# OpenResearchInstitute/ka9q-sdr

Measured on AMD Instinct MI355X. Metric: input Msamples/s + channels @ real-time, 16384-pt overlap-save, higher is better.
Workload: dtype f32

## Files before the change

### ka9q_sdr_amd/csrc/kq_demod64.hip

```cpp
#include "kq_device.hpp"
#include <cstdlib>
#include "kq_ldsfft.hpp"

namespace kq {

namespace {

__device__ __forceinline__ float2 shfl2(float2 v, int src) {
  return make_float2(__shfl(v.x, src, 64), __shfl(v.y, src, 64));
}
__device__ __forceinline__ float rdlane(float v, int src) {
  return __int_as_float(__builtin_amdgcn_readlane(__float_as_int(v), src));
}
__device__ __forceinline__ int bitrev6(int i) { return (int)(__brev((unsigned)i) >> 26); }

__device__ __forceinline__ void put_status(kq_chan_status &st, const Geom &g, const ChanDev &ch, const Planes &pl, int c, int b,
                                           int compute_n0, double n0_rate, float &n0) {
  st.if_power = pl.if_power[b];
  st.noise_gain = ch.noise_gain[c];
  st.plfreq = NAN;
  st.cphase = 0;
  st.pll_lock = 0;
  st.lock_count = 0;
  if (compute_n0) {
    float const fresh = pl.n0raw[(size_t)c * g.max_blocks + b];
    if (isnan(n0))
      n0 = fresh;
    else
      n0 = (float)((double)n0 + n0_rate * (double)(fresh - n0));
    st.n0 = n0;
  } else {
    st.n0 = NAN;
  }
}

template <class Op>
__device__ __forceinline__ float hreduce(float v, Op op) {
  int const lane = threadIdx.x & 63;
  v = op(v, lane_xor<16>(v, lane));
  v = op(v, lane_xor<8>(v, lane));
  v = op(v, lane_xor<4>(v, lane));
  v = op(v, lane_xor<2>(v, lane));
  v = op(v, lane_xor<1>(v, lane));
  return v;
}
__device__ __forceinline__ float hsum(float v) {
  return hreduce(v, [](float a, float b) { return a + b; });
}

template <bool FLAT>
__device__ void fm_channel_pair(const Geom &g, const ChanDev &ch, const Planes &pl, int c, int nblocks, int compute_n0) {
  int const lane = threadIdx.x & 63;
  int const h = lane >> 5, n = lane & 31;
  float const gain = ch.fm_gain[c];
  float const noise_gain = ch.noise_gain[c];
  int const kbin = bitrev6(lane);
  int const herm_src = bitrev6((64 - kbin) & 63);
  float2 HAf = make_float2(0.f, 0.f);
  if (!FLAT) {
    float2 const t = ch.aresp[(size_t)c * 33 + (kbin <= 32 ? kbin : 64 - kbin)];
    HAf = kbin <= 32 ? t : cconj(t);
  }
  bool const real_bin = kbin == 0 || kbin == 32;

  float2 wf[6], wi[6];
#pragma unroll
  for (int s = 0; s < 6; s++) {
    int const half = 1 << s;
    float sn, cs;
    sincospif((float)(lane & (half - 1)) / (float)half, &sn, &cs);
    wf[s] = make_float2(cs, -sn);
    wi[s] = make_float2(cs, sn);
  }

  float2 state = ch.fm_state[c];
  float lastaudio = ch.lastaudio[c];
  int sq = ch.sq_count[c];
  float foffset = ch.foffset[c], pdev = ch.pdev[c];
  float n0 = ch.n0[c];
  float hist = h ? 0.f : ch.ahist[(size_t)c * 32 + lane];
  float ifp_v = 0.f, n0raw_v = 0.f;
  const float2 *in = pl.filt + (size_t)c * g.max_blocks * 32;

  float2 s_next = (h < nblocks) ? in[lane] : make_float2(0.f, 0.f);
  for (int b = 0; b < nblocks; b += 2) {
    bool const have1 = b + 1 < nblocks;
    float2 const S = s_next;
    if (b + 2 < nblocks) s_next = (b + 2 + h < nblocks) ? in[(size_t)(b + 2) * 32 + lane] : make_float2(0.f, 0.f);
    if ((b & 63) == 0) {
      int const bb = b + lane;
      ifp_v = bb < nblocks ? pl.if_power[bb] : 0.f;
      n0raw_v = (compute_n0 && bb < nblocks) ? pl.n0raw[(size_t)c * g.max_blocks + bb] : 0.f;
    }

    float const t = cnrm(S);
    float const sum_t = hsum(t), sum_a = hsum(sqrtf(t));
    float const bbp = sum_t / 64.f;
    float const amp = (float)((double)sum_a / (M_SQRT2 * 32));
    float const variance = bbp - amp * amp;
    float snr = amp * amp / (2 * variance) - 1;
    snr = (0.0f > snr) ? 0.0f : snr;
    float const snr0 = rdlane(snr, 0), snr1 = rdlane(snr, 32);
    int nsq = sq + 1;
    nsq = nsq > 1000 ? 1000 : nsq;
    int const sq0 = (snr0 > 2) ? 0 : nsq;
    nsq = sq0 + 1;
    nsq = nsq > 1000 ? 1000 : nsq;
    int const sq1 = have1 ? ((snr1 > 2) ? 0 : nsq) : sq0;
    bool const open0 = sq0 < 2, open1 = have1 && sq1 < 2;
    bool const my_open = h ? open1 : open0;

    float const thr = (float)(0.55 * 0.55 * amp * amp);
    unsigned long long const raw = __ballot(t > thr);
    unsigned long long const m_lo = open0 ? (raw & 0xffffffffull) : 0ull;
    unsigned long long const m_hi = open1 ? (raw >> 32) : 0ull;
    unsigned long long const mask = m_lo | (m_hi << 32);
    bool const valid = (mask >> lane) & 1ull;
    unsigned long long const below = mask & ((1ull << lane) - 1ull);
    unsigned long long const upto = mask & ((2ull << lane) - 1ull);
    int const pv = below ? 63 - __clzll((long long)below) : -1;
    int const lv = upto ? 63 - __clzll((long long)upto) : -1;
    float2 const state_fb = (h && !open0) ? make_float2(0.f, 0.f) : state;
    float const la_fb = (h && !open0) ? 0.f : lastaudio;
    float2 const sp = shfl2(S, pv >= 0 ? pv : 0);
    float2 const stc = pv >= 0 ? cconj(sp) : state_fb;
    float2 const pr = cmul(S, stc);
    float const y = valid ? atan2f(pr.y, pr.x) : 0.f;
    float const yl = __shfl(y, lv >= 0 ? lv : 0, 64);
    float const out = my_open ? (lv >= 0 ? yl : la_fb) : 0.f;

    float const sum_y = hsum(out);
    float const vmax = hreduce((valid && n > 0) ? y : -INFINITY, [](float a, float b2) { return fmaxf(a, b2); });
    float const vmin = hreduce((valid && n > 0) ? y : INFINITY, [](float a, float b2) { return fminf(a, b2); });
    float const y_first = h ? rdlane(y, 32) : rdlane(y, 0);
    float const seed = ((mask >> (32 * h)) & 1ull) ? y_first : 0.f;
    float pdev_pos = fmaxf(seed, vmax), pdev_neg = fminf(seed, vmin);
    float const avg_f = sum_y / 32.f;
    pdev_pos -= avg_f;
    pdev_neg -= avg_f;
    float const mx = (pdev_pos > -pdev_neg) ? pdev_pos : -pdev_neg;
    float const fo_new = (float)(g.dsamprate * avg_f * (0.5 * M_1_PI));
    float const pd_new = (float)(g.dsamprate * mx * (0.5 * M_1_PI));
    float const fo0 = (sq0 < 1) ? rdlane(fo_new, 0) : foffset, pd0 = (sq0 < 1) ? rdlane(pd_new, 0) : pdev;
    float const fo1 = (have1 && sq1 < 1) ? rdlane(fo_new, 32) : fo0, pd1 = (have1 && sq1 < 1) ? rdlane(pd_new, 32) : pd0;

    {
      int const last0 = m_lo ? 63 - __clzll((long long)m_lo) : 0;
      int const last1 = m_hi ? 95 - __clzll((long long)m_hi) : 0;
      float2 const sl0 = cconj(make_float2(rdlane(S.x, last0), rdlane(S.y, last0)));
      float2 const sl1 = cconj(make_float2(rdlane(S.x, last1), rdlane(S.y, last1)));
      float const yl0 = rdlane(y, last0), yl1 = rdlane(y, last1);
      float2 st0 = open0 ? (m_lo ? sl0 : state) : make_float2(0.f, 0.f);
      float la0 = open0 ? (m_lo ? yl0 : lastaudio) : 0.f;
      if (have1) {
        st0 = open1 ? (m_hi ? sl1 : st0) : make_float2(0.f, 0.f);
        la0 = open1 ? (m_hi ? yl1 : la0) : 0.f;
      }
      state = st0;
      lastaudio = la0;
    }
    sq = sq1;
    foffset = fo1;
    pdev = pd1;

    float const xo = lane_xor<32>(out, lane);
    float a0 = out, a1 = xo;
    if (!FLAT) {
      float2 z = make_float2(h ? xo : hist, out);
#pragma unroll
      for (int s = 5; s >= 0; s--) {
        float2 const r = lane_xor_pow2(z, s, lane);
        z = ((lane >> s) & 1) ? cmul(csub(r, z), wf[s]) : cadd(z, r);
      }
      float2 const zm = cconj(shfl2(z, herm_src));
      float2 const z1 = make_float2(0.5f * (z.x + zm.x), 0.5f * (z.y + zm.y));
      float2 const z2 = make_float2(0.5f * (z.y - zm.y), -0.5f * (z.x - zm.x));
      float2 g1 = cmul(HAf, z1), g2 = cmul(HAf, z2);
      if (real_bin) g1.y = g2.y = 0.f;
      z = make_float2(g1.x - g2.y, g1.y + g2.x);
#pragma unroll
      for (int s = 0; s < 6; s++) {
        int const bit = (lane >> s) & 1;
        float2 const v = bit ? cmul(z, wi[s]) : z;
        float2 const r = lane_xor_pow2(v, s, lane);
        z = bit ? csub(r, v) : cadd(v, r);
      }
      a0 = z.x * gain;
      a1 = z.y * gain;
      if (h) {
        pl.audio[((size_t)c * g.max_blocks + b) * 64 + n] = a0;
        if (have1) pl.audio[((size_t)c * g.max_blocks + b + 1) * 64 + n] = a1;
      }
    } else {
      if (!h) {
        pl.audio[((size_t)c * g.max_blocks + b) * 64 + n] = a0;
        if (have1) pl.audio[((size_t)c * g.max_blocks + b + 1) * 64 + n] = a1;
      }
    }
    hist = have1 ? xo : out;

    float const ifp = h ? rdlane(ifp_v, (b + 1) & 63) : rdlane(ifp_v, b & 63);
    float const fresh0 = rdlane(n0raw_v, b & 63), fresh1 = rdlane(n0raw_v, (b + 1) & 63);
    float n0a = n0, n0b = n0;
    if (compute_n0) {
      n0a = isnan(n0) ? fresh0 : (float)((double)n0 + .01 * (double)(fresh0 - n0));
      n0b = have1 ? (isnan(n0a) ? fresh1 : (float)((double)n0a + .01 * (double)(fresh1 - n0a))) : n0a;
      n0 = n0b;
    }
    if (n == 0 && (h == 0 || have1)) {
      kq_chan_status rec;
      rec.if_power = ifp;
      rec.noise_gain = noise_gain;
      rec.plfreq = NAN;
      rec.cphase = 0;
      rec.pll_lock = 0;
      rec.lock_count = 0;
      rec.n0 = compute_n0 ? (h ? n0b : n0a) : NAN;
      rec.bb_power = bbp;
      rec.snr = snr;
      rec.foffset = h ? fo1 : fo0;
      rec.pdeviation = h ? pd1 : pd0;
      rec.agc_gain = 0;
      rec.squelch_count = h ? sq1 : sq0;
      rec.hangcount = 0;
      rec.blanked = my_open ? 32 - __popcll((mask >> (32 * h)) & 0xffffffffull) : 0;
      rec.nout = 32;
      pl.status[(size_t)c * g.max_blocks + b + h] = rec;
    }
  }
  if (!h) ch.ahist[(size_t)c * 32 + lane] = hist;
  if (lane == 0) {
    ch.fm_state[c] = state;
    ch.lastaudio[c] = lastaudio;
    ch.sq_count[c] = sq;
    ch.foffset[c] = foffset;
    ch.pdev[c] = pdev;
    ch.n0[c] = n0;
  }
}

__device__ void fm_channel_four_waves(const Geom &g, const ChanDev &ch, const Planes &pl, int c, int nblocks, int compute_n0) {
  __shared__ float2 s_S[2][64];
  __shared__ float s_a[2][2][4];
  __shared__ float s_out[2][64], s_y[2][64];
  __shared__ float s_b[2][2][5];
  __shared__ float2 s_z[2][64];
  __shared__ float s_c[2][2][6];
  int const lane = threadIdx.x & 63, role = threadIdx.x >> 6;
  int const h = lane >> 5, n = lane & 31;
  int const npairs = (nblocks + 1) / 2, niter = npairs + 3;

  if (role == 0) {
    int sq = ch.sq_count[c];
    const float2 *in = pl.filt + (size_t)c * g.max_blocks * 32;
    float2 s_next = (h < nblocks) ? in[lane] : make_float2(0.f, 0.f);
    for (int it = 0; it < niter; it++) {
      if (it < npairs) {
        int const b = 2 * it, par = it & 1;
        bool const have1 = b + 1 < nblocks;
        float2 const S = s_next;
        if (b + 2 < nblocks) s_next = (b + 2 + h < nblocks) ? in[(size_t)(b + 2) * 32 + lane] : make_float2(0.f, 0.f);
        float const t = cnrm(S);
        float const sum_t = hsum(t), sum_a = hsum(sqrtf(t));
        float const bbp = sum_t / 64.f;
        float const amp = (float)((double)sum_a / (M_SQRT2 * 32));
        float const variance = bbp - amp * amp;
        float snr = amp * amp / (2 * variance) - 1;
        snr = (0.0f > snr) ? 0.0f : snr;
        float const snr0 = rdlane(snr, 0), snr1 = rdlane(snr, 32);
        int nsq = sq + 1;
        nsq = nsq > 1000 ? 1000 : nsq;
        int const sq0 = (snr0 > 2) ? 0 : nsq;
        nsq = sq0 + 1;
        nsq = nsq > 1000 ? 1000 : nsq;
        int const sq1 = have1 ? ((snr1 > 2) ? 0 : nsq) : sq0;
        sq = sq1;
        s_S[par][lane] = S;
        if (n == 0) {
          float *st = s_a[par][h];
          st[0] = amp;
          st[1] = bbp;
          st[2] = snr;
          st[3] = __int_as_float(h ? sq1 : sq0);
        }
      }
      __syncthreads();
    }
    if (lane == 0) ch.sq_count[c] = sq;
    return;
  }

  if (role == 1) {
    float2 state = ch.fm_state[c];
    float lastaudio = ch.lastaudio[c];
    for (int it = 0; it < niter; it++) {
      if (it >= 1 && it - 1 < npairs) {
        int const b = 2 * (it - 1), par = (it - 1) & 1;
        bool const have1 = b + 1 < nblocks;
        float2 const S = s_S[par][lane];
        float const amp = s_a[par][h][0];
        int const sq0 = __float_as_int(s_a[par][0][3]), sq1 = __float_as_int(s_a[par][1][3]);
        bool const open0 = sq0 < 2, open1 = have1 && sq1 < 2;
        bool const my_open = h ? open1 : open0;
        float const t = cnrm(S);
        float const thr = (float)(0.55 * 0.55 * amp * amp);
        unsigned long long const raw = __ballot(t > thr);
        unsigned long long const m_lo = open0 ? (raw & 0xffffffffull) : 0ull;
        unsigned long long const m_hi = open1 ? (raw >> 32) : 0ull;
        unsigned long long const mask = m_lo | (m_hi << 32);
        bool const valid = (mask >> lane) & 1ull;
        unsigned long long const below = mask & ((1ull << lane) - 1ull);
        unsigned long long const upto = mask & ((2ull << lane) - 1ull);
        int const pv = below ? 63 - __clzll((long long)below) : -1;
        int const lv = upto ? 63 - __clzll((long long)upto) : -1;
        float2 const state_fb = (h && !open0) ? make_float2(0.f, 0.f) : state;
        float const la_fb = (h && !open0) ? 0.f : lastaudio;
        float2 const sp = shfl2(S, pv >= 0 ? pv : 0);
        float2 const stc = pv >= 0 ? cconj(sp) : state_fb;
        float2 const pr = cmul(S, stc);
        float const y = valid ? atan2f(pr.y, pr.x) : 0.f;
        float const yl = __shfl(y, lv >= 0 ? lv : 0, 64);
        float const out = my_open ? (lv >= 0 ? yl : la_fb) : 0.f;
        {
          int const last0 = m_lo ? 63 - __clzll((long long)m_lo) : 0;
          int const last1 = m_hi ? 95 - __clzll((long long)m_hi) : 0;
          float2 const sl0 = cconj(make_float2(rdlane(S.x, last0), rdlane(S.y, last0)));
          float2 const sl1 = cconj(make_float2(rdlane(S.x, last1), rdlane(S.y, last1)));
          float const yl0 = rdlane(y, last0), yl1 = rdlane(y, last1);
          float2 st0 = open0 ? (m_lo ? sl0 : state) : make_float2(0.f, 0.f);
          float la0 = open0 ? (m_lo ? yl0 : lastaudio) : 0.f;
          if (have1) {
            st0 = open1 ? (m_hi ? sl1 : st0) : make_float2(0.f, 0.f);
            la0 = open1 ? (m_hi ? yl1 : la0) : 0.f;
          }
          state = st0;
          lastaudio = la0;
        }
        s_out[par][lane] = out;
        s_y[par][lane] = y;
        if (n == 0) {
          float *st = s_b[par][h];
          st[0] = s_a[par][h][1];
          st[1] = s_a[par][h][2];
          st[2] = __int_as_float((int)(unsigned)(mask >> (32 * h)));
          st[3] = __int_as_float(h ? sq1 : sq0);
          st[4] = __int_as_float(my_open ? 32 - __popcll((mask >> (32 * h)) & 0xffffffffull) : 0);
        }
      }
      __syncthreads();
    }
    if (lane == 0) {
      ch.fm_state[c] = state;
      ch.lastaudio[c] = lastaudio;
    }
    return;
  }

  int const kbin = bitrev6(lane);
  if (role == 2) {
    int const herm_src = bitrev6((64 - kbin) & 63);
    float2 HAf;
    {
      float2 const t = ch.aresp[(size_t)c * 33 + (kbin <= 32 ? kbin : 64 - kbin)];
      HAf = kbin <= 32 ? t : cconj(t);
    }
    bool const real_bin = kbin == 0 || kbin == 32;
    float2 wf[6];
#pragma unroll
    for (int s = 0; s < 6; s++) {
      int const half = 1 << s;
      float sn, cs;
      sincospif((float)(lane & (half - 1)) / (float)half, &sn, &cs);
      wf[s] = make_float2(cs, -sn);
    }
    float foffset = ch.foffset[c], pdev = ch.pdev[c];
    float hist = h ? 0.f : ch.ahist[(size_t)c * 32 + lane];
    for (int it = 0; it < niter; it++) {
      if (it >= 2 && it - 2 < npairs) {
        int const b = 2 * (it - 2), par = (it - 2) & 1;
        bool const have1 = b + 1 < nblocks;
        float const out = s_out[par][lane], y = s_y[par][lane];
        unsigned const mask_h = (unsigned)__float_as_int(s_b[par][h][2]);
        int const sq0 = __float_as_int(s_b[par][0][3]), sq1 = __float_as_int(s_b[par][1][3]);
        bool const valid = (mask_h >> n) & 1u;
        float const sum_y = hsum(out);
        float const vmax = hreduce((valid && n > 0) ? y : -INFINITY, [](float a, float b2) { return fmaxf(a, b2); });
        float const vmin = hreduce((valid && n > 0) ? y : INFINITY, [](float a, float b2) { return fminf(a, b2); });
        float const y_first = h ? rdlane(y, 32) : rdlane(y, 0);
        float const seed = (mask_h & 1u) ? y_first : 0.f;
        float pdev_pos = fmaxf(seed, vmax), pdev_neg = fminf(seed, vmin);
        float const avg_f = sum_y / 32.f;
        pdev_pos -= avg_f;
        pdev_neg -= avg_f;
        float const mx = (pdev_pos > -pdev_neg) ? pdev_pos : -pdev_neg;
        float const fo_new = (float)(g.dsamprate * avg_f * (0.5 * M_1_PI));
        float const pd_new = (float)(g.dsamprate * mx * (0.5 * M_1_PI));
        float const fo0 = (sq0 < 1) ? rdlane(fo_new, 0) : foffset, pd0 = (sq0 < 1) ? rdlane(pd_new, 0) : pdev;
        float const fo1 = (have1 && sq1 < 1) ? rdlane(fo_new, 32) : fo0, pd1 = (have1 && sq1 < 1) ? rdlane(pd_new, 32) : pd0;
        foffset = fo1;
        pdev = pd1;

        float const xo = lane_xor<32>(out, lane);
        float2 z = make_float2(h ? xo : hist, out);
#pragma unroll
        for (int s = 5; s >= 0; s--) {
          float2 const r = lane_xor_pow2(z, s, lane);
          z = ((lane >> s) & 1) ? cmul(csub(r, z), wf[s]) : cadd(z, r);
        }
        float2 const zm = cconj(shfl2(z, herm_src));
        float2 const z1 = make_float2(0.5f * (z.x + zm.x), 0.5f * (z.y + zm.y));
        float2 const z2 = make_float2(0.5f * (z.y - zm.y), -0.5f * (z.x - zm.x));
        float2 g1 = cmul(HAf, z1), g2 = cmul(HAf, z2);
        if (real_bin) g1.y = g2.y = 0.f;
        s_z[par][lane] = make_float2(g1.x - g2.y, g1.y + g2.x);
        hist = have1 ? xo : out;
        if (n == 0) {
          float *st = s_c[par][h];
          st[0] = s_b[par][h][0];
          st[1] = s_b[par][h][1];
          st[2] = h ? fo1 : fo0;
          st[3] = h ? pd1 : pd0;
          st[4] = s_b[par][h][3];
          st[5] = s_b[par][h][4];
        }
      }
      __syncthreads();
    }
    if (!h) ch.ahist[(size_t)c * 32 + lane] = hist;
    if (lane == 0) {
      ch.foffset[c] = foffset;
      ch.pdev[c] = pdev;
    }
    return;
  }

  float const gain = ch.fm_gain[c];
  float const noise_gain = ch.noise_gain[c];
  float2 wi[6];
#pragma unroll
  for (int s = 0; s < 6; s++) {
    int const half = 1 << s;
    float sn, cs;
    sincospif((float)(lane & (half - 1)) / (float)half, &sn, &cs);
    wi[s] = make_float2(cs, sn);
  }
  float n0 = ch.n0[c];
  float ifp_v = 0.f, n0raw_v = 0.f;
  for (int it = 0; it < niter; it++) {
    if (it >= 3) {
      int const b = 2 * (it - 3), par = (it - 3) & 1;
      bool const have1 = b + 1 < nblocks;
      if ((b & 63) == 0) {
        int const bb = b + lane;
        ifp_v = bb < nblocks ? pl.if_power[bb] : 0.f;
        n0raw_v = (compute_n0 && bb < nblocks) ? pl.n0raw[(size_t)c * g.max_blocks + bb] : 0.f;
      }
      float2 z = s_z[par][lane];
#pragma unroll
      for (int s = 0; s < 6; s++) {
        int const bit = (lane >> s) & 1;
        float2 const v = bit ? cmul(z, wi[s]) : z;
        float2 const r = lane_xor_pow2(v, s, lane);
        z = bit ? csub(r, v) : cadd(v, r);
      }
      float const a0 = z.x * gain, a1 = z.y * gain;
      if (h) {
        pl.audio[((size_t)c * g.max_blocks + b) * 64 + n] = a0;
        if (have1) pl.audio[((size_t)c * g.max_blocks + b + 1) * 64 + n] = a1;
      }
      float const ifp = h ? rdlane(ifp_v, (b + 1) & 63) : rdlane(ifp_v, b & 63);
      float const fresh0 = rdlane(n0raw_v, b & 63), fresh1 = rdlane(n0raw_v, (b + 1) & 63);
      float n0a = n0, n0b = n0;
      if (compute_n0) {
        n0a = isnan(n0) ? fresh0 : (float)((double)n0 + .01 * (double)(fresh0 - n0));
        n0b = have1 ? (isnan(n0a) ? fresh1 : (float)((double)n0a + .01 * (double)(fresh1 - n0a))) : n0a;
        n0 = n0b;
      }
      if (n == 0 && (h == 0 || have1)) {
        const float *st = s_c[par][h];
        kq_chan_status rec;
        rec.if_power = ifp;
        rec.noise_gain = noise_gain;
        rec.plfreq = NAN;
        rec.cphase = 0;
        rec.pll_lock = 0;
        rec.lock_count = 0;
        rec.n0 = compute_n0 ? (h ? n0b : n0a) : NAN;
        rec.bb_power = st[0];
        rec.snr = st[1];
        rec.foffset = st[2];
        rec.pdeviation = st[3];
        rec.agc_gain = 0;
        rec.squelch_count = __float_as_int(st[4]);
        rec.hangcount = 0;
        rec.blanked = __float_as_int(st[5]);
        rec.nout = 32;
        pl.status[(size_t)c * g.max_blocks + b + h] = rec;
      }
    }
    __syncthreads();
  }
  if (lane == 0) ch.n0[c] = n0;
}

__device__ void fm_channel(const Geom &g, const ChanDev &ch, const Planes &pl, int c, int nblocks, int compute_n0) {
  if (ch.flags[c] & FLAG_FLAT)
    fm_channel_pair<true>(g, ch, pl, c, nblocks, compute_n0);
  else
    fm_channel_pair<false>(g, ch, pl, c, nblocks, compute_n0);
}

template <bool LINEAR, int OLEN, bool SPLIT>
__device__ void agc_channel(const Geom &g, const ChanDev &ch, const Planes &pl, int c, int nblocks, int compute_n0) {
  int const lane = threadIdx.x & 63;
  constexpr int BPI = 64 / OLEN;
  int const half = lane / OLEN, n = lane % OLEN;
  float const headroom = ch.headroom[c], recovery = ch.recovery[c];
  int const hangmax = ch.hangmax[c];
  bool const stereo = LINEAR && (ch.flags[c] & FLAG_STEREO) != 0;
  double const sh_ph = LINEAR ? ch.sh_phase[c] : 0.0, sh_f = LINEAR ? ch.sh_freq[c] : 0.0;
  float gain = ch.gain[c], dc = LINEAR ? 0.f : ch.dc[c];
  int hang = ch.hang[c];
  float n0 = ch.n0[c];
  const float2 *in = pl.filt + (size_t)c * g.max_blocks * OLEN;
  float2 s_next = (half < nblocks) ? in[lane] : make_float2(0.f, 0.f);
  __shared__ float s_hand[SPLIT ? 2 : 1][7][64];
  int const role = SPLIT ? (int)(threadIdx.x >> 6) : 0;
  int const niter = (nblocks + BPI - 1) / BPI;
  for (int it = 0; it < niter + (SPLIT ? 1 : 0); it++) {
    float2 S = make_float2(0.f, 0.f);
    float level = 0.f, env = 0.f, sig = 0.f, noi = 0.f, inv = 0.f;
    if (role == 0 && it < niter) {
      int const b0 = it * BPI;
      int const blk = b0 + half;
      int const nsamp = (b0 + BPI <= nblocks) ? 64 : OLEN;
      S = s_next;
      if (b0 + BPI < nblocks) s_next = (blk + BPI < nblocks) ? in[(size_t)(b0 + BPI) * OLEN + lane] : make_float2(0.f, 0.f);
      float const rp = S.x * S.x, ip = S.y * S.y;
      level = sqrtf(LINEAR ? rp + ip : S.x * S.x + S.y * S.y);
      env = level;
      sig = LINEAR ? rp : rp + ip;
      noi = LINEAR ? ip : 0.f;
      if (!LINEAR) sig = S.x * S.x + S.y * S.y;
#pragma unroll
      for (int o = OLEN / 2; o > 0; o >>= 1) {
        sig += __shfl_xor(sig, o, 64);
        noi += __shfl_xor(noi, o, 64);
      }
      if (!LINEAR) {
        float dc_mine = dc;
#pragma unroll 32
        for (int i = 0; i < nsamp; i++) {
          float const e = __builtin_bit_cast(float, __builtin_amdgcn_readlane(__builtin_bit_cast(int, env), i));
          dc += 0.0001f * (e - dc);
          dc_mine = (lane == i) ? dc : dc_mine;
        }
        level = dc_mine;
      }
      inv = headroom / level;
      if (SPLIT) {
        float(*hb)[64] = s_hand[it & 1];
        hb[0][lane] = S.x;
        hb[1][lane] = S.y;
        hb[2][lane] = level;
        hb[3][lane] = env;
        hb[4][lane] = sig;
        hb[5][lane] = noi;
        hb[6][lane] = inv;
      }
    }
    if (SPLIT) {
      if (role == 1 && it >= 1) {
        float(*hb)[64] = s_hand[(it - 1) & 1];
        S = make_float2(hb[0][lane], hb[1][lane]);
        level = hb[2][lane];
        env = hb[3][lane];
        sig = hb[4][lane];
        noi = hb[5][lane];
        inv = hb[6][lane];
      }
      __syncthreads();
      if (role == 0 || it == 0) continue;
    }
    int const b0 = (SPLIT ? it - 1 : it) * BPI;
    int const blk = b0 + half;
    bool const active = blk < nblocks;
    int const nsamp = (b0 + BPI <= nblocks) ? 64 : OLEN;
    float g_mine = gain;
    float gain_end[2] = {gain, gain};
    int hang_end[2] = {hang, hang};
    bool const held = !isnan(gain) && hang >= nsamp &&
                      __ballot(lane < nsamp && (LINEAR ? level * gain > headroom : gain * level > headroom)) == 0ull;
    if (held) {
      hang_end[0] = hang - OLEN;
      hang -= nsamp;
    }
    bool coast = false;
    if (!held && hangmax != 0 && hang < nsamp && !isnan(gain)) {
      float g = gain, after = gain;
#pragma unroll 32
      for (int i = 0; i < nsamp; i++) {
        g = (i >= hang) ? g * recovery : g;
        after = (lane == i) ? g : after;
      }
      float before = __shfl_up(after, 1, 64);
      before = (lane == 0) ? gain : before;
      coast = __ballot(lane < nsamp && (LINEAR ? level * before > headroom : before * level > headroom)) == 0ull;
      if (coast) {
        g_mine = after;
        gain_end[0] = __builtin_bit_cast(float, __builtin_amdgcn_readlane(__builtin_bit_cast(int, after), OLEN - 1));
        hang_end[0] = hang > OLEN ? hang - OLEN : 0;
        gain = g;
        hang = 0;
      }
// ... 305 lines not shown
```

### ka9q_sdr_amd/csrc/kq_full16k.hip

```cpp
#include "kq_device.hpp"
#include "kq_ldsfft.hpp"
#include <cmath>
#include <type_traits>

#include "kq_lane.hpp"
#include "kq_regfft.hpp"

#ifdef KQ_TIMELINE
__device__ unsigned long long kq_timeline[64][8][12];
#define KQ_STAMP(i)                                                                        \
  do {                                                                                     \
    __builtin_amdgcn_sched_barrier(0);                                                     \
    if (blockIdx.y == (gridDim.y > 40 ? 40 : gridDim.y / 2) && (blockIdx.x & 15) == 0 && (blockIdx.x >> 4) < 64 &&      \
        (threadIdx.x & 63) == 0)                                                           \
      kq_timeline[blockIdx.x >> 4][threadIdx.x >> 6][i] = clock64();                       \
    __builtin_amdgcn_sched_barrier(0);                                                     \
  } while (0)
extern "C" int kq_debug_timeline(unsigned long long *dst) {
  return hipMemcpyFromSymbol(dst, HIP_SYMBOL(kq_timeline), sizeof(kq_timeline)) == hipSuccess ? 0 : -1;
}
#else
#define KQ_STAMP(i)
#endif

// ... 314 lines not shown
          else if constexpr (K == 2)
            pk_cmul2(y[0], y[1], row(n1), ld2(sw + n1), row(n1 + 1), ld2(sw + n1 + 1));
          else
            y[0] = pk_cmul(row(n1), ld2(sw + n1));
        }
      };
      float const kbf = PLAIN == 2 ? (float)(2.0 * M_PI * 512.0 * r * (double)(t & 63)) : 0.f;
      v2f const kb = (v2f){kbf, kbf};
      v2f th = (v2f){0.f, 0.f};
      auto mix = [&](auto firstc, auto countc) {
        constexpr int n1 = decltype(firstc)::value, K = decltype(countc)::value;
        v2f y[4];
        mul(firstc, countc, y);
#pragma unroll
        for (int i = 0; i < K; i++) {
          if constexpr (PLAIN == 2) {
            th = th + kb;
            v2f z;
            asm("v_pk_fma_f32 %0, %1, %2, %3 op_sel:[1,0,0] op_sel_hi:[0,1,1] neg_lo:[0,1,0]" : "=v"(z) : "v"(y[i]), "v"(th), "v"(y[i]));
            row(n1 + i) = z;
          } else {
            row(n1 + i) = y[i];
          }
        }
      };
      using std::integral_constant;
      constexpr integral_constant<int, 1> k1{};
      constexpr integral_constant<int, 2> k2{};
      constexpr integral_constant<int, 4> k4{};
      mix(integral_constant<int, 1>{}, k1);
      mix(integral_constant<int, 2>{}, k2);
      mix(integral_constant<int, 4>{}, k4);
      mix(integral_constant<int, 8>{}, k4);
      mix(integral_constant<int, 12>{}, k4);
      mix(integral_constant<int, 16>{}, k4);
      mix(integral_constant<int, 20>{}, k2);
      mix(integral_constant<int, 22>{}, k2);
      mix(integral_constant<int, 24>{}, k4);
      mix(integral_constant<int, 28>{}, k4);
    } else if constexpr (!PLAIN) {
      OlderOsc older;
      load_older(ch, c, b * g.L, n_old > 0, older);
#pragma unroll
      for (int n1 = 0; n1 < 32; n1++) {
        int const i = 512 * n1 + t;
        double const m = mbase + i;
        bool const old = i < n_old;
        double pp = old ? hp0 : ph0, ff = old ? hf0 : f0, rr = old ? hr : r;
        pick_older(older, i, pp, ff, rr);
        double turns = pp + ff * m;
        if (rr != 0.0) turns += rr * (0.5 * m * (m - 1.0));
        v[rfft::bitrev5(n1)] = pk_cmul(buf_ld2(xr, toff, (unsigned)n1 * (unsigned)(512 * sizeof(float2))), phasor2(turns));
      }
    }
  }

  KQ_STAMP(1);
  __builtin_amdgcn_s_setprio(0);
  rfft::fft_dit_pk<32>(v);
  twiddle32(v, tlo, thi, pt);

  KQ_STAMP(2);
  v2f u[32];
  tw2[(t >> 5) * kTw2Pitch + (t & 31)] = make_float2(tw2_mine.x, tw2_mine.y);
#if defined(KQ_ABLATE) && (KQ_ABLATE & 1)
#pragma unroll
  for (int n2 = 0; n2 < 32; n2++) u[n2] = v[n2];
#else
  {
    int const rd = ((t >> 4) & 15) * kRow1 + (t & 15);
#pragma unroll
    for (int half = 0; half < 2; half++) {
#pragma unroll
      for (int k1 = 0; k1 < 16; k1++) xch[k1 * kRow1 + t] = make_float2(v[16 * half + k1].x, v[16 * half + k1].y);
#if !(defined(KQ_ABLATE) && (KQ_ABLATE & 4))
      __syncthreads();
#endif
      if ((t >> 8) == half) {
#pragma unroll
        for (int n2 = 0; n2 < 32; n2++) u[rfft::bitrev5(n2)] = ld2(xch + rd + 16 * n2);
      }
#if !(defined(KQ_ABLATE) && (KQ_ABLATE & 4))
      __syncthreads();
#endif
    }
  }
#endif

  KQ_STAMP(3);
  rfft::fft_dit_pk<32>(u);
  {
    const float4 *row = reinterpret_cast<const float4 *>(tw2 + (t & 15) * kTw2Pitch);
#pragma unroll
    for (int k2 = 0; k2 < 32; k2 += 4) {
      float4 const w = row[k2 / 2], x = row[k2 / 2 + 1];
      v2f const w0 = (v2f){w.x, w.y}, w1 = (v2f){w.z, w.w}, w2 = (v2f){x.x, x.y}, w3 = (v2f){x.z, x.w};
      if (k2) {
        pk_cmul4(u[k2], u[k2 + 1], u[k2 + 2], u[k2 + 3], u[k2], w0, u[k2 + 1], w1, u[k2 + 2], w2, u[k2 + 3], w3);
      } else {
        u[1] = pk_cmul(u[1], w1);
        pk_cmul2(u[2], u[3], u[2], w2, u[3], w3);
      }
    }
  }

  KQ_STAMP(4);
  v2f ya[16], yb[16];
#if defined(KQ_ABLATE) && (KQ_ABLATE & 2)
#pragma unroll
  for (int n3 = 0; n3 < 16; n3++) {
    ya[n3] = u[n3];
    yb[n3] = u[16 + n3];
  }
#else
  {
    int const wr = (t & 15) * kRow2 + ((t >> 4) & 15) * kCol2;
    int const rd = (t >> 5) * kCol2 + (t & 31);
#pragma unroll
    for (int half = 0; half < 2; half++) {
      if ((t >> 8) == half) {
#pragma unroll
        for (int k2 = 0; k2 < 32; k2++) xch[wr + k2] = make_float2(u[k2].x, u[k2].y);
      }
#if !(defined(KQ_ABLATE) && (KQ_ABLATE & 4))
      __syncthreads();
#endif
#pragma unroll
      for (int n3 = 0; n3 < 16; n3++) (half ? yb : ya)[rfft::bitrev4(n3)] = ld2(xch + n3 * kRow2 + rd);
#if !(defined(KQ_ABLATE) && (KQ_ABLATE & 4))
      __syncthreads();
#endif
    }
  }
#endif

  KQ_STAMP(5);
  rfft::fft_dit_pk<16>(ya);
  rfft::fft_dit_pk<16>(yb);
  int const ka = full16k_bin(t), kb = ka + kFull16kHalf;

  if (DUMP && c == spec_ch) {
    float2 *o = spec_dump + (size_t)b * kNfull;
    constexpr int kStep = BIG ? 4 : 1;
#pragma unroll
    for (int k3 = 0; k3 < 16; k3++) {
      o[kStep * (ka + 1024 * k3) + r4] = make_float2(ya[k3].x, ya[k3].y);
      o[kStep * (kb + 1024 * k3) + r4] = make_float2(yb[k3].x, yb[k3].y);
    }
  }

  KQ_STAMP(6);
  float2 *Xs = xch;
  float2 *G = Xs + Ndec;
  auto to_f2 = [](v2f a) { return make_float2(a.x, a.y); };
  if constexpr (BIG != 0) {
    float2 *const Xg = big.xs + ((size_t)c * g.max_blocks + b) * Ndec;
    auto put = [&](int q, v2f val) {
      int const k = 4 * q + r4;
      if (k <= Ndec / 2)
        Xg[k] = to_f2(val);
      else if (k > kNfull - Ndec / 2)
        Xg[k - kNfull + Ndec] = to_f2(val);
    };
    if (Ndec <= 4096) {
      put(ka, ya[0]);
      put(kb, yb[0]);
      put(ka + 15 * 1024, ya[15]);
      put(kb + 15 * 1024, yb[15]);
    } else {
#pragma unroll
      for (int k3 = 0; k3 < 16; k3++) {
        put(ka + 1024 * k3, ya[k3]);
        put(kb + 1024 * k3, yb[k3]);
      }
    }
  } else if (Ndec <= 1024) {
    if (ka <= Ndec / 2) Xs[ka] = to_f2(ya[0]);
    if (kb <= Ndec / 2) Xs[kb] = to_f2(yb[0]);
    if (ka + 15 * 1024 > kN - Ndec / 2) Xs[ka - 1024 + Ndec] = to_f2(ya[15]);
    if (kb + 15 * 1024 > kN - Ndec / 2) Xs[kb - 1024 + Ndec] = to_f2(yb[15]);
  } else {
#pragma unroll
    for (int k3 = 0; k3 < 16; k3++) {
      if (1024 * k3 > Ndec / 2 && 1024 * k3 + 1023 <= kN - Ndec / 2) continue;
#pragma unroll
      for (int half = 0; half < 2; half++) {
        int const n = (half ? kb : ka) + 1024 * k3;
        float2 const val = to_f2(half ? yb[k3] : ya[k3]);
        if (n <= Ndec / 2)
          Xs[n] = val;
        else if (n > kN - Ndec / 2)
          Xs[n - kN + Ndec] = val;
      }
    }
  }
  const float2 *H = ch.resp + (size_t)c * Ndec;
  bool const isb = (ch.fflags[c] & FLAG_ISB) != 0;
  v2f epi_h = {0.f, 0.f}, epi_h2 = {0.f, 0.f}, epi_w[5] = {};
  bool const epi64 = BIG == 0 && (EPI == 1 || (EPI == 0 && Ndec == 64));
  if (epi64 && t < 64) {
    int const q = (int)(__brev((unsigned)t) >> 26);
    epi_h = ld2(H + q);
    if (isb) epi_h2 = ld2(H + ((64 - q) & 63));
#pragma unroll
    for (int st = 0; st < 5; st++) epi_w[st] = buf_ld2(tabr, (unsigned)t * 8u, (unsigned)(kTabEpi + st * 64) * 8u);
  }
  int const epiR = (BIG == 0 && (EPI == 2 || (EPI == 0 && Ndec >= 128 && Ndec <= 512))) ? Ndec >> 6 : 0;
  v2f epi_post = {1.f, 0.f};
  if (epiR && t < 64 * epiR) {
    int const r = t >> 6, l = t & 63;
    int const q = (int)(__brev((unsigned)l) >> 26);
    int const k = epiR * q + r;
    epi_h = ld2(H + k);
    if (isb) epi_h2 = ld2(H + ((Ndec - k) & (Ndec - 1)));
#pragma unroll
    for (int st = 0; st < 5; st++) epi_w[st] = buf_ld2(tabr, (unsigned)l * 8u, (unsigned)(kTabEpi + st * 64) * 8u);
    float sn, cs;
    sincospif(2.f * (float)(r * l) / (float)Ndec, &sn, &cs);
    epi_post = (v2f){cs, sn};
  }

  bool n0_fast = false;
  int outside = 0;
  if constexpr (N0) {
    v2f pp[16];
    typedef const unsigned long long __attribute__((address_space(4))) *lane_masks;
    int const ns = __builtin_amdgcn_readfirstlane(ch.n0slot[c]);
    lane_masks const lm = (lane_masks)(
        ch.n0lane + ((size_t)(ns * (BIG ? 4 : 1) + r4) * (kT / 64) + __builtin_amdgcn_readfirstlane(t >> 6)) * 32);
#pragma unroll
    for (int k3 = 0; k3 < 16; k3++) {
      float p0, p1;
      asm("v_mul_f32 %0, %1, %1" : "=v"(p0) : "v"(ya[k3].x));
      asm("v_mul_f32 %0, %1, %1" : "=v"(p1) : "v"(yb[k3].x));
      asm("v_fma_f32 %0, %1, %1, %0" : "+v"(p0) : "v"(ya[k3].y));
      asm("v_fma_f32 %0, %1, %1, %0" : "+v"(p1) : "v"(yb[k3].y));
      asm("v_cndmask_b32_e64 %0, 0, %0, %1" : "+v"(p0) : "s"(lm[k3]));
      asm("v_cndmask_b32_e64 %0, 0, %0, %1" : "+v"(p1) : "s"(lm[16 + k3]));
      pp[k3] = (v2f){p0, p1};
    }
    outside = (int)ch.n0meta[ns * (BIG ? 4 : 1) + r4];
    v2f s2;
    {
      v2f const a0 = pp[0] + pp[1], a1 = pp[2] + pp[3], a2 = pp[4] + pp[5], a3 = pp[6] + pp[7];
      v2f const a4 = pp[8] + pp[9], a5 = pp[10] + pp[11], a6 = pp[12] + pp[13], a7 = pp[14] + pp[15];
      s2 = ((a0 + a1) + (a2 + a3)) + ((a4 + a5) + (a6 + a7));
    }
    float const tot = wave_sum_to63(s2.x + s2.y);
    if ((t & 63) == 63) red_f[0][t >> 6] = tot;
    __syncthreads();
    float total = 0;
#pragma unroll
    for (int k = 0; k < kT / 64; k++) total += red_f[0][k];
    int bins1 = outside;
    unsigned long long *const slots = BIG ? big.sync + ((size_t)c * g.max_blocks + b) * 12 : nullptr;
    if constexpr (BIG != 0) {
      sibling_exchange(slots, r4, __float_as_uint(total), big.epoch, sib_f, big.err);
      total = (sib_f[0] + sib_f[1]) + (sib_f[2] + sib_f[3]);
      const unsigned *const mt = ch.n0meta + ns * 4;
      bins1 = (int)(mt[0] + mt[1] + mt[2] + mt[3]);
    }
    float const thr = (total / bins1) * 2;
    n0_fast = total < INFINITY && thr < INFINITY && thr >= 1e-26f;
    if (n0_fast) {
      int const e = (__float_as_int(thr) >> 23) & 0xff;
      float const scale = __int_as_float((127 + 40 + 127 - e) << 23);
      float const cs = thr * scale;
      v2f const nsc = (v2f){-scale, -scale}, c2 = (v2f){cs, cs};
      v2f acc_e = (v2f){0.f, 0.f}, acc_o = acc_e, cnt_e = acc_e, cnt_o = acc_e;
#pragma unroll
      for (int k3 = 0; k3 < 16; k3++) {
        v2f keep;
        asm("v_pk_fma_f32 %0, %1, %2, %3 clamp" : "=v"(keep) : "v"(nsc), "v"(pp[k3]), "v"(c2));
        if (k3 & 1) {
          acc_o = rfft::pk_fma(keep, pp[k3], acc_o);
          cnt_o += keep;
        } else {
          acc_e = rfft::pk_fma(keep, pp[k3], acc_e);
          cnt_e += keep;
        }
      }
      v2f const acc2 = acc_e + acc_o, cnt2 = cnt_e + cnt_o;
      float const acc = wave_sum_to63(acc2.x + acc2.y), cnt = wave_sum_to63(cnt2.x + cnt2.y);
      if ((t & 63) == 63) {
        red_f[1][t >> 6] = acc;
        red_c[t >> 6] = cnt;
      }
    } else {
      {
        float const inf = INFINITY;
#pragma unroll
        for (int k3 = 0; k3 < 16; k3++) {
          asm("v_cndmask_b32_e64 %0, %2, %0, %1" : "+v"(pp[k3].x) : "s"(lm[k3]), "v"(inf));
          asm("v_cndmask_b32_e64 %0, %2, %0, %1" : "+v"(pp[k3].y) : "s"(lm[16 + k3]), "v"(inf));
        }
      }
      float avg = INFINITY;
      float tf_last = 0;
      int bins_last = 0;
      asm volatile("" : "+v"(avg));
      for (int iter = 0; iter < 2; iter++) {
        float acc = 0;
        int wave_bins = 0;
        float const th = avg * 2;
#pragma unroll
        for (int k3 = 0; k3 < 16; k3++) {
          bool const ta = pp[k3].x < th, tb = pp[k3].y < th;
          acc += ta ? pp[k3].x : 0.f;
          acc += tb ? pp[k3].y : 0.f;
          wave_bins += __popcll(__ballot(ta)) + __popcll(__ballot(tb));
        }
        acc = wave_sum(acc);
        __syncthreads();
        if ((t & 63) == 0) {
          red_f[iter][t >> 6] = acc;
          red_i[iter][t >> 6] = wave_bins;
        }
        __syncthreads();
        float tf = 0;
        int bins = 0;
#pragma unroll
        for (int k = 0; k < kT / 64; k++) {
          tf += red_f[iter][k];
          bins += red_i[iter][k];
        }
        if (BIG != 0 && iter == 0) {
          sibling_exchange(slots + 4, r4, __float_as_uint(tf), big.epoch, sib_f + 4, big.err);
          sibling_exchange(slots + 8, r4, (unsigned)bins, big.epoch, sib_f + 8, big.err);
          tf = (sib_f[4] + sib_f[5]) + (sib_f[6] + sib_f[7]);
          bins = (int)(__float_as_uint(sib_f[8]) + __float_as_uint(sib_f[9]) + __float_as_uint(sib_f[10]) + __float_as_uint(sib_f[11]));
        }
        avg = tf / bins;
        tf_last = tf;
        bins_last = bins;
      }
      if constexpr (BIG != 0) {
        if (t == 0) big.n0part[((size_t)c * g.max_blocks + b) * 4 + r4] = make_float2(tf_last, (float)bins_last);
      } else {
        if (t == 0) pl.n0raw[(size_t)c * g.max_blocks + b] = (float)(avg / (2.0 * kN * g.samprate));
      }
    }
  }

  KQ_STAMP(7);
  __syncthreads();
  KQ_STAMP(8);
  if (N0 && n0_fast && t == kT - 64) {
    float tf = 0, bins = 0;
#pragma unroll
    for (int k = 0; k < kT / 64; k++) {
      tf += red_f[1][k];
      bins += red_c[k];
    }
    bins -= (float)(kN - outside);
    if constexpr (BIG != 0) {
      big.n0part[((size_t)c * g.max_blocks + b) * 4 + r4] = make_float2(tf, bins);
    } else {
      float const avg = tf / bins;
      pl.n0raw[(size_t)c * g.max_blocks + b] = (float)(avg / (2.0 * kN * g.samprate));
    }
  }
  if (big.iir.sums != nullptr && blockIdx.x == 0 && blockIdx.y == 0 && t >= kT - 64)
    block_energy_iir_wave(big.iir.sums, big.iir.split, big.iir.update, big.iir.nblocks, big.iir.L, big.iir.state, big.iir.if_power,
                          t & 63);
  if constexpr (BIG != 0) return;
  if (epi64) {
    if (t >= 64) return;
    int const q = (int)(__brev((unsigned)t) >> 26);
    v2f z = pk_cmul(epi_h, ld2(Xs + q));
    if (isb && q != 0 && q != 32) {
      v2f const other = pk_cmul(epi_h2, ld2(Xs + 64 - q));
      v2f const oc = (v2f){other.x, -other.y};
      z = q < 32 ? z + oc : z - oc;
    }
    auto stage = [&](auto mm, v2f w, bool first) {
      constexpr int half = decltype(mm)::value;
      v2f const v = first ? z : pk_cmul(z, w);
      v2f const r = (v2f){lane_xor<half>(v.x, t), lane_xor<half>(v.y, t)};
      float const sg = __int_as_float(0x3f800000 | ((t & half) ? 0x80000000 : 0));
      z = rfft::pk_fma(v, (v2f){sg, sg}, r);
    };
    stage(std::integral_constant<int, 1>{}, z, true);
    stage(std::integral_constant<int, 2>{}, epi_w[0], false);
    stage(std::integral_constant<int, 4>{}, epi_w[1], false);
    stage(std::integral_constant<int, 8>{}, epi_w[2], false);
    stage(std::integral_constant<int, 16>{}, epi_w[3], false);
    stage(std::integral_constant<int, 32>{}, epi_w[4], false);
    float2 *o = pl.filt + ((size_t)c * g.max_blocks + b) * g.olen;
    if (t >= 64 - g.olen) o[t - (64 - g.olen)] = make_float2(z.x, z.y);
    KQ_STAMP(9);
    return;
  }
  if (epiR) {
    float2 *Z = G;
    if (t < 64 * epiR) {
      int const r = t >> 6, l = t & 63;
      int const q = (int)(__brev((unsigned)l) >> 26);
      int const k = epiR * q + r;
      v2f z = pk_cmul(epi_h, ld2(Xs + k));
      if (isb && k != 0 && 2 * k != Ndec) {
        v2f const other = pk_cmul(epi_h2, ld2(Xs + Ndec - k));
        v2f const oc = (v2f){other.x, -other.y};
        z = 2 * k < Ndec ? z + oc : z - oc;
      }
      auto stage = [&](auto mm, v2f w, bool first) {
        constexpr int half = decltype(mm)::value;
        v2f const v = first ? z : pk_cmul(z, w);
        v2f const rr = (v2f){lane_xor<half>(v.x, l), lane_xor<half>(v.y, l)};
        float const sg = __int_as_float(0x3f800000 | ((l & half) ? 0x80000000 : 0));
        z = rfft::pk_fma(v, (v2f){sg, sg}, rr);
      };
      stage(std::integral_constant<int, 1>{}, z, true);
      stage(std::integral_constant<int, 2>{}, epi_w[0], false);
      stage(std::integral_constant<int, 4>{}, epi_w[1], false);
      stage(std::integral_constant<int, 8>{}, epi_w[2], false);
      stage(std::integral_constant<int, 16>{}, epi_w[3], false);
      stage(std::integral_constant<int, 32>{}, epi_w[4], false);
      z = pk_cmul(z, epi_post);
      Z[64 * r + l] = make_float2(z.x, z.y);
    }
    __syncthreads();
    if (t >= 64) return;
    float2 *o = pl.filt + ((size_t)c * g.max_blocks + b) * g.olen;
    int const first = Ndec - g.olen;
    auto combine = [&](auto rc) {
      constexpr int R = decltype(rc)::value;
      constexpr int bits = R == 2 ? 1 : R == 4 ? 2 : 3;
      float2 v[R];
#pragma unroll
      for (int r = 0; r < R; r++) {
        float2 const zz = Z[64 * r + t];
        v[(int)(__brev((unsigned)r) >> (32 - bits))] = make_float2(zz.x, -zz.y);
      }
      rfft::fft_dit<R>(v);
#pragma unroll
      for (int j = 0; j < R; j++) {
        int const i = t + 64 * j - first;
        if (i >= 0 && i < g.olen) o[i] = make_float2(v[j].x, -v[j].y);
      }
    };
    if (epiR == 2)
      combine(std::integral_constant<int, 2>{});
    else if (epiR == 4)
      combine(std::integral_constant<int, 4>{});
    else
      combine(std::integral_constant<int, 8>{});
    KQ_STAMP(9);
    return;
  }
  if constexpr (EPI != 0) return;
  for (int p = t; p <= Ndec / 2; p += kT) {
    float2 gp = cmul(H[p], Xs[p]);
    if (p > 0 && p < Ndec / 2) {
      int const k = Ndec - p;
      float2 gn = cmul(H[k], Xs[k]);
      if (isb) {
        float2 const pos = gp, neg = gn;
        gp = cadd(pos, cconj(neg));
        gn = csub(neg, cconj(pos));
      }
      G[bitrev((unsigned)k, g.log2Ndec)] = gn;
    }
    G[bitrev((unsigned)p, g.log2Ndec)] = gp;
  }
  lds_fft<+1>(G, g.log2Ndec, tw, g.tw_log2);

  float2 *o = pl.filt + ((size_t)c * g.max_blocks + b) * g.olen;
  for (int i = t; i < g.olen; i += kT) o[i] = G[Ndec - g.olen + i];
  KQ_STAMP(9);
}

__global__ void k_epilogue64k(Geom g, ChanDev ch, Planes pl, const float2 *__restrict__ tw, Big64 big,
                              const int *__restrict__ chan_list, int compute_n0) {
  extern __shared__ __attribute__((aligned(16))) float2 G[];
  int const t = threadIdx.x, Ndec = g.Ndec;
  int const c = chan_list ? chan_list[blockIdx.x] : (int)blockIdx.x, b = blockIdx.y;
  size_t const cb = (size_t)c * g.max_blocks + b;
  if (compute_n0 && t == 0) {
    const float2 *p = big.n0part + cb * 4;
    float const tf = (p[0].x + p[1].x) + (p[2].x + p[3].x), bins = (p[0].y + p[1].y) + (p[2].y + p[3].y);
    float const avg = tf / bins;
    pl.n0raw[cb] = (float)(avg / (2.0 * 65536.0 * g.samprate));
  }
  const float2 *Xs = big.xs + cb * Ndec;
  const float2 *H = ch.resp + (size_t)c * Ndec;
  bool const isb = (ch.fflags[c] & FLAG_ISB) != 0;
  for (int p = t; p <= Ndec / 2; p += blockDim.x) {
    float2 gp = cmul(H[p], Xs[p]);
    if (p > 0 && p < Ndec / 2) {
      int const k = Ndec - p;
      float2 gn = cmul(H[k], Xs[k]);
      if (isb) {
        float2 const pos = gp, neg = gn;
        gp = cadd(pos, cconj(neg));
        gn = csub(neg, cconj(pos));
      }
      G[bitrev((unsigned)k, g.log2Ndec)] = gn;
    }
    G[bitrev((unsigned)p, g.log2Ndec)] = gp;
  }
  lds_fft<+1>(G, g.log2Ndec, tw, g.tw_log2);
  float2 *o = pl.filt + cb * g.olen;
  for (int i = t; i < g.olen; i += blockDim.x) o[i] = G[Ndec - g.olen + i];
}

__global__ void __launch_bounds__(256) k_full16k_rows(ChanDev ch, int nchan) {
  int const i = (int)(blockIdx.x * blockDim.x + threadIdx.x);
  if (i >= 32 * nchan) return;
  ch.row_ph[i] = row_phasor(ch.lo_freq[i >> 5], i & 31);
}
void launch_full16k_rows(hipStream_t s, const ChanDev &ch, int nchan) {
  if (nchan > 0 && ch.row_ph) hipLaunchKernelGGL(k_full16k_rows, dim3((32 * nchan + 255) / 256), dim3(256), 0, s, ch, nchan);
}

bool full16k_supported(const Geom &g) {
  return g.N == kN && 2 * g.Ndec <= kXchElems && g.Ndec >= 4;
}

static const float2 *twiddle_tables() {
  return (const float2 *)upload_once(TABLE_FULL16K, kN, kTabSize * sizeof(float2), [](void *bytes) {
    float2 *h = (float2 *)bytes;
    auto w = [](long long e) {
      double const ang = -2.0 * M_PI * (double)(e % kN) / kN;
// ... 116 lines not shown
```

Baseline: 394,700.

## Micro-tune demod and 16k FFT epilogue: scalar loads, fma cmul, uniform branches

```diff
diff --git a/ka9q_sdr_amd/csrc/kq_demod64.hip b/ka9q_sdr_amd/csrc/kq_demod64.hip
--- a/ka9q_sdr_amd/csrc/kq_demod64.hip
+++ b/ka9q_sdr_amd/csrc/kq_demod64.hip
@@ -13,6 +13,32 @@
   return __int_as_float(__builtin_amdgcn_readlane(__float_as_int(v), src));
 }
 __device__ __forceinline__ int bitrev6(int i) { return (int)(__brev((unsigned)i) >> 26); }
+
+template <int R, int I>
+__device__ __forceinline__ float2 cmul_as(float2 a, float2 b) {
+#pragma clang fp contract(off)
+  float re, im;
+  if (R == 1) {
+    float const t = a.y * b.y;
+    re = __builtin_fmaf(a.x, b.x, -t);
+  } else {
+    float const t0 = a.x * b.x, t1 = a.y * b.y;
+    re = t0 - t1;
+  }
+  if (I == 0) {
+    float const t = a.x * b.y;
+    im = __builtin_fmaf(a.y, b.x, t);
+  } else {
+    float const t = a.y * b.x;
+    im = __builtin_fmaf(a.x, b.y, t);
+  }
+  return make_float2(re, im);
+}
+__device__ __forceinline__ float2 cmul_fwd_stage(float2 d, float2 w, int s) {
+  return s == 5 ? cmul_as<2, 0>(d, w) : cmul_as<1, 1>(d, w);
+}
+__device__ __forceinline__ float2 cmul_response(float2 h, float2 z) { return cmul_as<1, 0>(h, z); }
+__device__ __forceinline__ float2 cmul_inv_stage(float2 z, float2 w) { return cmul_as<1, 0>(z, w); }
 
 __device__ __forceinline__ void put_status(kq_chan_status &st, const Geom &g, const ChanDev &ch, const Planes &pl, int c, int b,
                                            int compute_n0, double n0_rate, float &n0) {
@@ -170,18 +196,18 @@
 #pragma unroll
       for (int s = 5; s >= 0; s--) {
         float2 const r = lane_xor_pow2(z, s, lane);
-        z = ((lane >> s) & 1) ? cmul(csub(r, z), wf[s]) : cadd(z, r);
+        z = ((lane >> s) & 1) ? cmul_fwd_stage(csub(r, z), wf[s], s) : cadd(z, r);
       }
       float2 const zm = cconj(shfl2(z, herm_src));
       float2 const z1 = make_float2(0.5f * (z.x + zm.x), 0.5f * (z.y + zm.y));
       float2 const z2 = make_float2(0.5f * (z.y - zm.y), -0.5f * (z.x - zm.x));
-      float2 g1 = cmul(HAf, z1), g2 = cmul(HAf, z2);
+      float2 g1 = cmul_response(HAf, z1), g2 = cmul_response(HAf, z2);
       if (real_bin) g1.y = g2.y = 0.f;
       z = make_float2(g1.x - g2.y, g1.y + g2.x);
 #pragma unroll
       for (int s = 0; s < 6; s++) {
         int const bit = (lane >> s) & 1;
-        float2 const v = bit ? cmul(z, wi[s]) : z;
+        float2 const v = bit ? cmul_inv_stage(z, wi[s]) : z;
         float2 const r = lane_xor_pow2(v, s, lane);
         z = bit ? csub(r, v) : cadd(v, r);
       }
@@ -405,12 +431,12 @@
 #pragma unroll
         for (int s = 5; s >= 0; s--) {
           float2 const r = lane_xor_pow2(z, s, lane);
-          z = ((lane >> s) & 1) ? cmul(csub(r, z), wf[s]) : cadd(z, r);
+          z = ((lane >> s) & 1) ? cmul_fwd_stage(csub(r, z), wf[s], s) : cadd(z, r);
         }
         float2 const zm = cconj(shfl2(z, herm_src));
         float2 const z1 = make_float2(0.5f * (z.x + zm.x), 0.5f * (z.y + zm.y));
         float2 const z2 = make_float2(0.5f * (z.y - zm.y), -0.5f * (z.x - zm.x));
-        float2 g1 = cmul(HAf, z1), g2 = cmul(HAf, z2);
+        float2 g1 = cmul_response(HAf, z1), g2 = cmul_response(HAf, z2);
         if (real_bin) g1.y = g2.y = 0.f;
         s_z[par][lane] = make_float2(g1.x - g2.y, g1.y + g2.x);
         hist = have1 ? xo : out;
@@ -459,7 +485,7 @@
 #pragma unroll
       for (int s = 0; s < 6; s++) {
         int const bit = (lane >> s) & 1;
-        float2 const v = bit ? cmul(z, wi[s]) : z;
+        float2 const v = bit ? cmul_inv_stage(z, wi[s]) : z;
         float2 const r = lane_xor_pow2(v, s, lane);
         z = bit ? csub(r, v) : cadd(v, r);
       }
diff --git a/ka9q_sdr_amd/csrc/kq_full16k.hip b/ka9q_sdr_amd/csrc/kq_full16k.hip
--- a/ka9q_sdr_amd/csrc/kq_full16k.hip
+++ b/ka9q_sdr_amd/csrc/kq_full16k.hip
@@ -490,6 +490,7 @@
   KQ_STAMP(6);
   float2 *Xs = xch;
   float2 *G = Xs + Ndec;
+  int const wv = __builtin_amdgcn_readfirstlane(t >> 6);
   auto to_f2 = [](v2f a) { return make_float2(a.x, a.y); };
   if constexpr (BIG != 0) {
     float2 *const Xg = big.xs + ((size_t)c * g.max_blocks + b) * Ndec;
@@ -513,10 +514,12 @@
       }
     }
   } else if (Ndec <= 1024) {
-    if (ka <= Ndec / 2) Xs[ka] = to_f2(ya[0]);
-    if (kb <= Ndec / 2) Xs[kb] = to_f2(yb[0]);
-    if (ka + 15 * 1024 > kN - Ndec / 2) Xs[ka - 1024 + Ndec] = to_f2(ya[15]);
-    if (kb + 15 * 1024 > kN - Ndec / 2) Xs[kb - 1024 + Ndec] = to_f2(yb[15]);
+    int const hd = Ndec / 2;
+    float2 *const lo = Xs + ka, *const hi = lo + (Ndec - 1024);
+    if (ka <= hd) lo[0] = to_f2(ya[0]);
+    if (ka <= hd - kFull16kHalf) lo[kFull16kHalf] = to_f2(yb[0]);
+    if (ka > 1024 - hd) hi[0] = to_f2(ya[15]);
+    if (ka > 1024 - kFull16kHalf - hd) hi[kFull16kHalf] = to_f2(yb[15]);
   } else {
 #pragma unroll
     for (int k3 = 0; k3 < 16; k3++) {
@@ -533,10 +536,20 @@
     }
   }
   const float2 *H = ch.resp + (size_t)c * Ndec;
-  bool const isb = (ch.fflags[c] & FLAG_ISB) != 0;
-  v2f epi_h = {0.f, 0.f}, epi_h2 = {0.f, 0.f}, epi_w[5] = {};
+  typedef const int __attribute__((address_space(4))) *chan_words;
+  int const cu = __builtin_amdgcn_readfirstlane(c);
+  int const isb_word = ((chan_words)ch.fflags)[cu] & FLAG_ISB;
+  auto isb_now = [&]() {
+    int w = isb_word;
+    asm("" : "+s"(w));
+    return w != 0;
+  };
+  bool const isb = isb_now();
+  v2f epi_h, epi_h2, epi_w[5];
+  asm("" : "=v"(epi_h), "=v"(epi_h2));
+  asm("" : "=v"(epi_w[0]), "=v"(epi_w[1]), "=v"(epi_w[2]), "=v"(epi_w[3]), "=v"(epi_w[4]));
   bool const epi64 = BIG == 0 && (EPI == 1 || (EPI == 0 && Ndec == 64));
-  if (epi64 && t < 64) {
+  if (epi64 && wv == 0) {
     int const q = (int)(__brev((unsigned)t) >> 26);
     epi_h = ld2(H + q);
     if (isb) epi_h2 = ld2(H + ((64 - q) & 63));
@@ -563,9 +576,8 @@
   if constexpr (N0) {
     v2f pp[16];
     typedef const unsigned long long __attribute__((address_space(4))) *lane_masks;
-    int const ns = __builtin_amdgcn_readfirstlane(ch.n0slot[c]);
-    lane_masks const lm = (lane_masks)(
-        ch.n0lane + ((size_t)(ns * (BIG ? 4 : 1) + r4) * (kT / 64) + __builtin_amdgcn_readfirstlane(t >> 6)) * 32);
+    int const ns = ((chan_words)ch.n0slot)[cu];
+    lane_masks const lm = (lane_masks)(ch.n0lane + ((size_t)(ns * (BIG ? 4 : 1) + r4) * (kT / 64) + wv) * 32);
 #pragma unroll
     for (int k3 = 0; k3 < 16; k3++) {
       float p0, p1;
@@ -585,11 +597,12 @@
       s2 = ((a0 + a1) + (a2 + a3)) + ((a4 + a5) + (a6 + a7));
     }
     float const tot = wave_sum_to63(s2.x + s2.y);
-    if ((t & 63) == 63) red_f[0][t >> 6] = tot;
+    bool const last_lane = (t & 63) == 63;
+    if (last_lane) red_f[0][wv] = tot;
     __syncthreads();
-    float total = 0;
-#pragma unroll
-    for (int k = 0; k < kT / 64; k++) total += red_f[0][k];
+    float total = red_f[0][0];
+#pragma unroll
+    for (int k = 1; k < kT / 64; k++) total += red_f[0][k];
     int bins1 = outside;
     unsigned long long *const slots = BIG ? big.sync + ((size_t)c * g.max_blocks + b) * 12 : nullptr;
     if constexpr (BIG != 0) {
@@ -604,13 +617,24 @@
       int const e = (__float_as_int(thr) >> 23) & 0xff;
       float const scale = __int_as_float((127 + 40 + 127 - e) << 23);
       float const cs = thr * scale;
-      v2f const nsc = (v2f){-scale, -scale}, c2 = (v2f){cs, cs};
-      v2f acc_e = (v2f){0.f, 0.f}, acc_o = acc_e, cnt_e = acc_e, cnt_o = acc_e;
+      v2f sc2, c2;
+      sc2.x = scale;
+      c2.x = cs;
+      asm("" : "=v"(sc2.y), "=v"(c2.y));
+      v2f acc_e, acc_o, cnt_e, cnt_o;
 #pragma unroll
       for (int k3 = 0; k3 < 16; k3++) {
         v2f keep;
-        asm("v_pk_fma_f32 %0, %1, %2, %3 clamp" : "=v"(keep) : "v"(nsc), "v"(pp[k3]), "v"(c2));
-        if (k3 & 1) {
+        asm("v_pk_fma_f32 %0, %1, %2, %3 op_sel_hi:[0,1,0] neg_lo:[1,0,0] neg_hi:[1,0,0] clamp"
+            : "=v"(keep)
+            : "v"(sc2), "v"(pp[k3]), "v"(c2));
+        if (k3 == 0) {
+          acc_e = keep * pp[k3];
+          cnt_e = keep;
+        } else if (k3 == 1) {
+          acc_o = keep * pp[k3];
+          cnt_o = keep;
+        } else if (k3 & 1) {
           acc_o = rfft::pk_fma(keep, pp[k3], acc_o);
           cnt_o += keep;
         } else {
@@ -620,9 +644,9 @@
       }
       v2f const acc2 = acc_e + acc_o, cnt2 = cnt_e + cnt_o;
       float const acc = wave_sum_to63(acc2.x + acc2.y), cnt = wave_sum_to63(cnt2.x + cnt2.y);
-      if ((t & 63) == 63) {
-        red_f[1][t >> 6] = acc;
-        red_c[t >> 6] = cnt;
+      if (last_lane) {
+        red_f[1][wv] = acc;
+        red_c[wv] = cnt;
       }
     } else {
       {
@@ -647,6 +671,7 @@
           acc += ta ? pp[k3].x : 0.f;
           acc += tb ? pp[k3].y : 0.f;
           wave_bins += __popcll(__ballot(ta)) + __popcll(__ballot(tb));
+          asm volatile("" : "+s"(wave_bins));
         }
         acc = wave_sum(acc);
         __syncthreads();
@@ -684,9 +709,9 @@
   __syncthreads();
   KQ_STAMP(8);
   if (N0 && n0_fast && t == kT - 64) {
-    float tf = 0, bins = 0;
-#pragma unroll
-    for (int k = 0; k < kT / 64; k++) {
+    float tf = red_f[1][0], bins = red_c[0];
+#pragma unroll
+    for (int k = 1; k < kT / 64; k++) {
       tf += red_f[1][k];
       bins += red_c[k];
     }
@@ -703,10 +728,12 @@
                           t & 63);
   if constexpr (BIG != 0) return;
   if (epi64) {
-    if (t >= 64) return;
+    int wv_now = wv;
+    asm("" : "+s"(wv_now));
+    if (wv_now != 0) return;
     int const q = (int)(__brev((unsigned)t) >> 26);
     v2f z = pk_cmul(epi_h, ld2(Xs + q));
-    if (isb && q != 0 && q != 32) {
+    if (isb_now() && q != 0 && q != 32) {
       v2f const other = pk_cmul(epi_h2, ld2(Xs + 64 - q));
       v2f const oc = (v2f){other.x, -other.y};
       z = q < 32 ? z + oc : z - oc;
```

Result: faster. 399,200, median of 6 (+1.2%).
